# filodb/FiloDB

Measured on NVIDIA H100. Metric: samples/s scanned+aggregated (rate over 10M series); % HBM roofline, higher is better.
Workload: dtype f64

## Files before the change

filodb_b200/csrc/capi.cu:

```cuda
#include "../../include/filo_b200.h"
#include "kernels.h"
#include "host_util.h"
#include "scan_tile_layout.h"
#include "scan_wp_layout.h"
#include <cub/cub.cuh>
#include <algorithm>
#include <atomic>
#include <chrono>
#include <cmath>
#include <cstdio>
#include <cstdlib>
#include <cstring>
#include <mutex>
#include <string>
#include <thread>
#include <vector>

using namespace filo;

struct filo_ctx {
  int device = 0;
  filo_cfg cfg{};
  cudaStream_t stream = nullptr;
  int sm_count = 132;
// ... 776 lines not shown
  CUDA_TRY(ctx, tmp.alloc((void**)&d_err, 16)); CUDA_TRY(ctx, tmp.alloc((void**)&d_counters, 16));
  CUDA_TRY(ctx, cudaMemsetAsync(d_err, 0, 16, s)); CUDA_TRY(ctx, cudaMemsetAsync(d_counters, 0, 16, s));
  EventPair evp;
  if (stats) { CUDA_TRY(ctx, cudaEventCreate(&evp.e0)); CUDA_TRY(ctx, cudaEventCreate(&evp.e1)); }
  cudaEvent_t& e0 = evp.e0; cudaEvent_t& e1 = evp.e1;

  const uint32_t acc_bytes = fused ? align_up((uint32_t)q.T * (moments ? 20u : 12u), 128) : 0;
  const bool need_corr2 = need_corr && t->any_drop;
  uint32_t scratch2 = align_up((uint32_t)t->max_chunks * (uint32_t)CHUNK_DESC_BYTES, 16) +
                      ((uint32_t)t->max_rows + (uint32_t)t->max_chunks * 8u) * 8u * (1u + (t->any_nonconst_ts ? 1u : 0u) + (need_corr2 ? 1u : 0u));
  scratch2 = align_up(scratch2 + 16, 128);
  const uint32_t rec_cap = align_up(t->max_rec_bytes + 16, 128);
  const size_t per_warp2 = v2_smem_per_warp(rec_cap, scratch2, acc_bytes);
  const char* force_env = std::getenv("FILO_KERNEL");
  const std::string force = force_env ? force_env : "";
  const size_t smem_cap = std::min<size_t>(ctx->max_smem_optin, 227 * 1024);
  const bool use_v2 = force != "v1" && t->max_rec_bytes > 0 && per_warp2 * FAST_WARPS + 1024 <= smem_cap;
  const int64_t work = fused ? t->n_items : t->n_series;
  int64_t launches = 0;
  uint8_t* gscratch = nullptr;
  ScanLaunch L{t->d_arena, t->d_rec_off, t->n_series, q, nullptr, 0, 0, d_counters, d_err, 1, s};
  uint32_t rec_cap_used = 0;
  if (use_v2) {
    const size_t cta_smem = per_warp2 * FAST_WARPS + 1024;
    const int ctas_per_sm = (int)std::max<size_t>(1, std::min<size_t>(64 / FAST_WARPS, (size_t)(228 * 1024) / cta_smem));
    L.grid = (int)std::max<int64_t>(1, std::min<int64_t>((work + FAST_WARPS - 1) / FAST_WARPS, (int64_t)ctx->sm_count * ctas_per_sm));
    L.scratch_bytes = scratch2; L.use_smem = 1; rec_cap_used = rec_cap;
  } else {
    uint32_t scratch = align_up((uint32_t)t->max_chunks * (uint32_t)CHUNK_DESC_BYTES, 16) + (uint32_t)t->max_rows * 8u * (need_corr ? 3u : 2u);
    scratch = align_up(scratch + 16, 16);
    const size_t cta_smem = (size_t)(scratch + acc_bytes) * SCAN_WARPS;
    const int use_smem = cta_smem <= std::min<size_t>(ctx->max_smem_optin, 200 * 1024);
    int ctas_per_sm = 16;
    if (use_smem) ctas_per_sm = (int)std::max<size_t>(1, std::min<size_t>(16, (size_t)(220 * 1024) / std::max<size_t>(cta_smem + 1024, 1)));
    L.grid = (int)std::max<int64_t>(1, std::min<int64_t>((work + SCAN_WARPS - 1) / SCAN_WARPS, (int64_t)ctx->sm_count * ctas_per_sm));
    if (!use_smem) CUDA_TRY(ctx, tmp.alloc((void**)&gscratch, (size_t)L.grid * SCAN_WARPS * (scratch + acc_bytes)));
    L.gscratch = gscratch; L.scratch_bytes = scratch; L.use_smem = use_smem;
  }
  const int fn_cls = fn_class_of(fn, q.cumulative, q.long_values);
  const uint64_t wrows = (uint64_t)(q.window / q.step) + 1;
  TileSmem TL{};
  bool use_tile = false;
  if (use_v2 && force != "v2" && fn_cls == CLASS_SUM && t->n_series > 0) {
    TL = tile_layout(t->max_rec_bytes, (uint32_t)t->max_rows, (uint32_t)q.T, (uint32_t)std::min<uint64_t>(2 * wrows, 1u << 20) + 16);
    if (((size_t)TL.total + 1024) * 2 > (size_t)228 * 1024) TL = tile_layout(t->max_rec_bytes, (uint32_t)t->max_rows, (uint32_t)q.T, 16);
    use_tile = (size_t)TL.total + 1024 <= smem_cap;
  }
  WpSmem WL{};
  bool use_wp = false;
  if (use_tile && force != "v3" && wrows <= 4096 && t->max_chunks > 0) {
    const bool alias = wp_max_items((uint32_t)t->max_chunks, (uint32_t)q.T, (uint32_t)wrows) <= 64;
    WL = wp_layout(t->max_rec_bytes, (uint32_t)t->max_rows, (uint32_t)t->max_chunks, (uint32_t)q.T, (uint32_t)wrows, alias);
    WL.warps = (uint32_t)std::min<size_t>(smem_cap / WL.per_warp, alias ? WP_MAX_WARPS_ALIAS : WP_MAX_WARPS);
    use_wp = WL.warps >= 4;
  }
  WpCtrSmem WC{};
  bool use_wp_ctr = false;
  if (use_v2 && force != "v2" && force != "v3" && fn_cls == CLASS_COUNTER && t->n_series > 0 && t->max_chunks > 0 &&
      (!fused || q.T <= TILE_AGG_ACC * TILE_THREADS) && wp_ctr_tile_footprint_ok(t->max_rec_bytes, (uint32_t)t->max_rows, (uint32_t)q.T, smem_cap)) {
    WC = wp_ctr_layout(t->max_rec_bytes, (uint32_t)t->max_rows, (uint32_t)t->max_chunks, (uint32_t)q.T, fused, t->any_nonconst_ts, moments);
    const size_t w = std::min<size_t>((smem_cap - sizeof(TileCtrTab) * (TILE_CTR_TABMAX + 1) - 64) / WC.per_warp, WC.tsr != 0 ? 16 : WP_CTR_MAX_WARPS);
    WC.warps = (uint32_t)w; WC.tab = (uint32_t)(WC.per_warp * w);
    use_wp_ctr = w >= 4;
  }
  auto run_per_series = [&](double* outp) -> int32_t {
    if (use_tile || use_wp_ctr) {
      int64_t* d_list = nullptr; unsigned long long* d_cnt = nullptr;
      CUDA_TRY(ctx, tmp.alloc((void**)&d_list, (size_t)t->n_series * 8));
      CUDA_TRY(ctx, tmp.alloc((void**)&d_cnt, 16));
      CUDA_TRY(ctx, cudaMemsetAsync(d_cnt, 0, 16, s));
      ScanLaunch LT = L;
      static const bool dbg = std::getenv("FILO_DEBUG_SYNC") != nullptr;
      if (use_wp) {
        LT.grid = (int)std::max<int64_t>(1, std::min<int64_t>((t->n_series + WL.warps - 1) / WL.warps, (int64_t)ctx->sm_count));
        CUDA_TRY(ctx, launch_scan_wp(LT, outp, WL, d_list, d_cnt));
      } else if (use_wp_ctr) {
        LT.grid = (int)std::max<int64_t>(1, std::min<int64_t>((t->n_series + WC.warps - 1) / WC.warps, (int64_t)ctx->sm_count));
        CUDA_TRY(ctx, launch_scan_wp_ctr(LT, outp, WC, d_list, d_cnt));
      } else {
        const int ctas_per_sm = ((size_t)TL.total + 1024) * 2 <= (size_t)228 * 1024 ? 2 : 1;
        const int64_t n_tiles = (t->n_series + TILE_NS - 1) / TILE_NS;
        LT.grid = (int)std::max<int64_t>(1, std::min<int64_t>(n_tiles, (int64_t)ctx->sm_count * ctas_per_sm));
        if (dbg) { fprintf(stderr, "[filo] tile kernel fn=%d T=%d grid=%d smem=%u pitch=%u\n", fn, q.T, LT.grid, TL.total, TL.vals_pitch); fflush(stderr); }
        CUDA_TRY(ctx, launch_scan_tile(LT, outp, TL, d_list, d_cnt));
      }
      if (dbg) { CUDA_TRY(ctx, cudaStreamSynchronize(s)); fprintf(stderr, "[filo] tile kernel done\n"); fflush(stderr); }
      ScanLaunch LF = L; LF.list = d_list; LF.list_count = d_cnt;
      CUDA_TRY(ctx, launch_scan_series_v2(LF, outp, rec_cap_used));
      if (dbg) { CUDA_TRY(ctx, cudaStreamSynchronize(s)); fprintf(stderr, "[filo] fallback kernel done\n"); fflush(stderr); }
      launches += 2;
    } else {
      CUDA_TRY(ctx, use_v2 ? launch_scan_series_v2(L, outp, rec_cap_used) : launch_scan_series(L, outp));
      launches += 1;
    }
    return FILO_OK;
  };
  if (stats) CUDA_TRY(ctx, cudaEventRecord(e0, s));
  if (agg == FILO_AGG_NONE) {
    { int32_t rc = run_per_series((double*)d_out_values); if (rc) return rc; }
  } else if (!fused) {
    double* per = nullptr;
    CUDA_TRY(ctx, tmp.alloc((void**)&per, (size_t)t->n_series * q.T * 8));
    { int32_t rc = run_per_series(per); if (rc) return rc; }
    CUDA_TRY(ctx, launch_topk(per, t->grouped ? t->d_order : nullptr, t->d_group_start, t->n_groups, q.T, k, agg == FILO_AGG_BOTTOMK,
                              (double*)d_out_values, (int64_t*)d_out_aux, s));
    launches += 1;
// ... 541 lines not shown
```

filodb_b200/csrc/scan_wp.cuh:

```cuda
#pragma once
#include "scan_tile.cuh"
#include "scan_wp_layout.h"

namespace filo {

#ifdef FILO_CUSIM
__device__ __forceinline__ uint32_t wp_soff(const void* p) { return (uint32_t)(reinterpret_cast<const uint8_t*>(p) - smem); }
__device__ __forceinline__ uint32_t wp_lds32(uint32_t off) { uint32_t v; std::memcpy(&v, smem + off, 4); return v; }
#else
__device__ __forceinline__ uint32_t wp_soff(const void* p) { return smem_u32(p); }
__device__ __forceinline__ uint32_t wp_lds32(uint32_t off) { uint32_t v; asm volatile("ld.shared.u32 %0, [%1];" : "=r"(v) : "r"(off)); return v; }
#endif

#if defined(FILO_WP_PROF) && !defined(FILO_CUSIM)
__device__ unsigned long long g_wp_prof[16];
#define WPROF_DECL uint32_t wpp_t0 = (uint32_t)clock(), wpp_acc[14] = {0, 0, 0, 0, 0, 0, 0, 0, 0, 0, 0, 0, 0, 0};
#define WPROF(i) { const uint32_t wpp_t1 = (uint32_t)clock(); wpp_acc[i] += wpp_t1 - wpp_t0; wpp_t0 = wpp_t1; }
#define WPROF_COUNT(i) { ++wpp_acc[i]; }
#define WPROF_FLUSH if (lane == 0) { for (int wpp_i = 0; wpp_i < 14; ++wpp_i) atomicAdd(&g_wp_prof[wpp_i], (unsigned long long)wpp_acc[wpp_i]); atomicAdd(&g_wp_prof[15], 1ull); }
#else
#define WPROF_DECL
#define WPROF(i)
#define WPROF_COUNT(i)
#define WPROF_FLUSH
// ... 237 lines not shown

constexpr uint32_t WP_FINAL = 0, WP_RAWFIN = 1, WP_JUNC = 2, WP_GAP = 3;
__device__ __forceinline__ int wp_chunk_of(const WpChunk* CD, int n, int k) {
  int ci = -1;
  for (int c = 0; c < n; ++c) if (CD[c].nblk > 0 && k >= CD[c].kT0) ci = c;
  return ci;
}
__device__ __forceinline__ uint32_t wp_class(const WpChunk* CD, int n, int k, uint32_t& jslot) {
  const int ci = wp_chunk_of(CD, n, k);
  jslot = 0;
  if (ci < 0 || k > CD[ci].kT1) return WP_GAP;
  const WpChunk& ch = CD[ci];
  const int i = k - ch.kT0;
  if (i < ch.jzb * WP_R) { jslot = (uint32_t)(ch.joff + i) | (i < ch.hs ? 128u : 0u); return WP_JUNC; }
  return i >= ch.tb * WP_R ? WP_RAWFIN : WP_FINAL;
}
__device__ __forceinline__ int wp_rows_in(const WpChunk& x, int k, int Wr) {
  int lo = x.s0 + k; if (lo < 0) lo = 0; int hi = x.s0 + k + Wr; if (hi > x.nrows - 1) hi = x.nrows - 1;
  return hi - lo + 1;
}

__device__ __forceinline__ void wp_item(const WpChunk* CD, const WpSmem& L, int it, int items, int psi, int& pp, int& op, int& inf) {
  const bool active = it < items;
  int ci = 0;
  if (CD[1].nblk > 0 && it >= CD[1].blk0) ci = 1;
  if (CD[2].nblk > 0 && it >= CD[2].blk0) ci = 2;
  if (CD[3].nblk > 0 && it >= CD[3].blk0) ci = 3;
  const WpChunk& ch = CD[ci];
  const int b = active ? it - ch.blk0 : 0;
  const int k0 = ch.kT0 + WP_R * b;
  pp = ch.vidx0 + 9 * b;
  const bool tojz = b < ch.jzb;
  const bool raw = tojz || b >= ch.tb;
  op = tojz ? (int)WP_OFF_J + 8 * (ch.joff + WP_R * b) : (int)L.out + 8 * (k0 + ((k0 + psi) >> 3));
  int jEnd = !active ? -1 : tojz ? WP_R - 1 : ch.kT1 - k0;
  if (jEnd > WP_R - 1) jEnd = WP_R - 1;
  const int ot = tojz ? 0 : (k0 + psi) & 7;
  inf = (jEnd + 1) | ((raw ? 1 : 0) << 4) | (ot << 5) | (ci << 8) | (k0 << 10);
}

template <int FN, int NW>
__global__ void __launch_bounds__(NW * 32, 1)
scan_wp_sum_kernel(const uint8_t* __restrict__ arena, const int64_t* __restrict__ rec_off, int64_t n_series, QueryParams q,
                   double* __restrict__ out, WpSmem L, int64_t* __restrict__ fallback_list, unsigned long long* __restrict__ fallback_count,
                   unsigned long long* d_counters, int* d_err) {
  extern __shared__ __align__(128) uint8_t smem[];
  const unsigned FULL = 0xffffffffu;
  const int lane = threadIdx.x & 31, warp = threadIdx.x >> 5;
  uint8_t* wb = smem + (size_t)warp * L.per_warp;
  uint64_t* bar = reinterpret_cast<uint64_t*>(wb);
  WpChunk* CD = reinterpret_cast<WpChunk*>(wb + WP_OFF_DESC);
  uint64_t* xtab = reinterpret_cast<uint64_t*>(wb + WP_OFF_J);
  double* J = reinterpret_cast<double*>(wb + WP_OFF_J);
  uint8_t* R = wb + WP_OFF_REC;
  double* V = reinterpret_cast<double*>(wb + L.vals);
  double* O = reinterpret_cast<double*>(wb + L.out);
  const int64_t nwarps = (int64_t)gridDim.x * (blockDim.x >> 5);
  int64_t s = (int64_t)blockIdx.x * (blockDim.x >> 5) + warp;
  if (lane == 0) { mbar_init(bar, 1); mbar_fence_init(); }
  __syncwarp();

  int64_t winDur = q.inclusive ? q.window : q.window - 1; if (winDur < 0) winDur = 0;
  const double fdiv = (double)(q.inclusive ? winDur : winDur + 1), frcp = 1.0 / fdiv;
  const int64_t S0 = q.start - winDur, E0 = q.start;
  const int64_t lastEnd = q.start + (int64_t)(q.T - 1) * q.step;
  StepDiv sd; sd.init(q.step);
  const double NaNv = __longlong_as_double(0x7ff8000000000000LL);

  int64_t m_init = 0, m_end = 0; int m_nrows = -1, m_n = -1, m_wire = -1; bool m_ok = false;
  int dd_dst[2] = {0, 0}, dd_inf[2] = {0, 0}, wi_pp[2] = {0, 0}, wi_op[2] = {0, 0}, wi_inf[2] = {0, 0};
  int gz[3] = {-1, -1, -1}; bool gz_all = true;
  int p_Wr = 0, p_items = 0, p_nfull = 0, p_psi = 0; double p_rcpn = 0.0; bool p_oal = false;
  uint32_t p_cls = 0; uint64_t p_jx = 0;
  int64_t rows_scanned = 0, bytes_scanned = 0;
  uint32_t parity = 0;

  auto issue = [&](int64_t off, uint32_t sz) {
    mbar_expect_tx(bar, sz);
    tma_load_1d(R, arena + off, sz, bar);
  };
  int64_t cur_off = 0; uint32_t cur_sz = 0;
  if (s < n_series) { cur_off = rec_off[s]; cur_sz = (uint32_t)(rec_off[s + 1] - cur_off); }
  if (s < n_series && cur_sz <= L.rec_cap && lane == 0) issue(cur_off, cur_sz);
  WPROF_DECL

  for (; s < n_series; s += nwarps) {
    const int64_t sn = s + nwarps;
    int64_t nxt_off = 0; uint32_t nxt_end = 0;
    if (sn < n_series) { nxt_off = rec_off[sn]; nxt_end = (uint32_t)rec_off[sn + 1]; }
    const bool staged = cur_sz <= L.rec_cap;
    WPROF_COUNT(10)
    WPROF(9)
    if (staged) { mbar_wait(bar, parity); parity ^= 1; }
    WPROF(0)
    const WpParsed P = wp_parse<true>(R, q, staged, lane);
    const uint32_t nxt_sz = nxt_end - (uint32_t)nxt_off;
    WPROF(1)
    bool regular = P.regular;
    const bool have = P.have; const int n = P.n, c = lane;
    const int64_t init = P.init, end_time = P.end_time;
    const int nrows = P.nrows, num_rows = P.num_rows, vbytes = P.vbytes, ng = P.ng, vwire = P.vwire, grp_base = P.grp_base, ngroups = P.ngroups;
    const uint32_t voff = P.voff, w12 = P.w12; const bool any_raw = P.any_raw;
    const bool samec = !(c < n) || (init == m_init && nrows == m_nrows && end_time == m_end && vwire == m_wire);
    const bool same_all = __all_sync(FULL, samec);
    const bool same = m_ok && n == m_n && same_all;
    if (regular && !same) {
      WPROF_COUNT(11)
      m_init = init; m_end = end_time; m_nrows = nrows; m_n = n; m_wire = vwire; m_ok = false;
      int64_t s0 = 0, e0 = 0;
      if (have) { s0 = sd.ceil_div(S0 - init); e0 = sd.floor_div(E0 - init); }
      const int Wr = (int)(e0 - s0);
      int64_t kT0 = -e0; if (kT0 < 0) kT0 = 0;
      int64_t kT1 = (int64_t)(nrows - 1) - s0; if (kT1 > q.T - 1) kT1 = q.T - 1;
      const bool touch = have && kT0 <= kT1;
      if (!touch) { kT0 = 0x3fffffff; kT1 = -1; }
      const int Wr0 = __shfl_sync(FULL, Wr, 0);
      bool okp = !have || Wr == Wr0;
      if (Wr0 < 8 || (uint32_t)Wr0 + 1 > L.jcap) okp = false;
      const unsigned tm = __ballot_sync(FULL, touch) & 0xfu;
      if (tm != 0) { const unsigned lowbit = tm & (0u - tm); const unsigned filled = tm + lowbit; if ((filled & (filled - 1)) != 0) okp = false; }
      const int64_t kT1p = __shfl_up_sync(FULL, kT1, 1), kT1pp = __shfl_up_sync(FULL, kT1, 2), kT0n = __shfl_down_sync(FULL, kT0, 1);
      const bool prev_t = c > 0 && ((tm >> (c - 1)) & 1u), next_t = c + 1 < WP_MAXC && ((tm >> (c + 1)) & 1u);
      if (touch && c >= 2 && ((tm >> (c - 2)) & 1u) && !(kT1pp < kT0)) okp = false;
      int64_t ownLo = kT0, ownHi = kT1;
      if (touch && prev_t && kT1p + 1 > ownLo) ownLo = kT1p + 1;
      if (touch && next_t && kT0n - 1 < ownHi) ownHi = kT0n - 1;
      const int hs = touch ? (int)(ownLo - kT0) : 0;
      const int nblk = touch ? (int)((kT1 - kT0 + WP_R) / WP_R) : 0;
      const int jzb = (hs + WP_R - 1) / WP_R;
      const int tb = (touch && ownHi < kT1) ? (int)((ownHi + 1 - kT0) / WP_R) : nblk;
      if (touch && jzb > tb) okp = false;
      int blk0, items, joff, jtot;
      { const int a0 = __shfl_sync(FULL, nblk, 0), a1 = __shfl_sync(FULL, nblk, 1), a2 = __shfl_sync(FULL, nblk, 2), a3 = __shfl_sync(FULL, nblk, 3);
        blk0 = (c > 0 ? a0 : 0) + (c > 1 ? a1 : 0) + (c > 2 ? a2 : 0); items = a0 + a1 + a2 + a3; }
      { const int z = jzb * WP_R;
        const int a0 = __shfl_sync(FULL, z, 0), a1 = __shfl_sync(FULL, z, 1), a2 = __shfl_sync(FULL, z, 2), a3 = __shfl_sync(FULL, z, 3);
        joff = (c > 0 ? a0 : 0) + (c > 1 ? a1 : 0) + (c > 2 ? a2 : 0); jtot = a0 + a1 + a2 + a3; }
      if ((uint32_t)jtot > L.jcap) okp = false;
      if (L.alias && items > 64) okp = false;
      const int fr = touch ? (int)(s0 + kT0) : 0;
      int rowpos = 0;
      {
        int base = 0;
#pragma unroll
        for (int cc = 0; cc < WP_MAXC; ++cc) {
          int x;
// ... 17 lines not shown
          p_psi = (-(int)__shfl_sync(FULL, (int)(touch ? kT0 : 0), first_t)) & 7;
          p_oal = __all_sync(FULL, !touch || (((int)kT0 + p_psi) & 7) == 0); }
        p_Wr = Wr0; p_items = items; p_nfull = Wr0 + 1; p_rcpn = 1.0 / (double)(Wr0 + 1);
        __syncwarp();
        {
          int tot = 0;
          gz[0] = gz[1] = gz[2] = -1;
          for (int g = 0; g <= n; ++g) {
            const int g0 = g == 0 ? 0 : CD[g - 1].rowpos + CD[g - 1].nrows;
            const int g1 = g == n ? pend : CD[g].rowpos;
#pragma unroll
            for (int u = 0; u < 3; ++u) { const int i = u * 32 + lane - tot; if (i >= 0 && i < g1 - g0) gz[u] = wp_vidx(g0 + i); }
            tot += g1 - g0;
          }
          gz_all = tot <= 96;
        }
        {
          uint32_t cls = 0; uint64_t jx = 0; int nj = 0;
#pragma unroll 1
          for (int m = 0; m < 16 && lane + 32 * m < q.T; ++m) {
            uint32_t js;
            const uint32_t code = wp_class(CD, n, lane + 32 * m, js);
            cls |= code << (2 * m);
            if (code == WP_JUNC) { jx |= (uint64_t)js << (8 * nj); ++nj; }
          }
          p_cls = cls; p_jx = jx;
        }
        {
          const int gb1 = __shfl_sync(FULL, have ? grp_base : 0x7fffffff, 1), gb2 = __shfl_sync(FULL, have ? grp_base : 0x7fffffff, 2),
                    gb3 = __shfl_sync(FULL, have ? grp_base : 0x7fffffff, 3);
#pragma unroll
          for (int jj = 0; jj < 2; ++jj) {
            const int slot = jj * 32 + lane;
            const bool active = slot < ngroups;
            const int ci = active ? (slot >= gb1 ? 1 : 0) + (slot >= gb2 ? 1 : 0) + (slot >= gb3 ? 1 : 0) : 0;
            const int gbc = ci == 0 ? 0 : ci == 1 ? gb1 : ci == 2 ? gb2 : gb3;
            const int g = active ? slot - gbc : 0;
            const int pq = CD[ci].rowpos + 1 + g * 8;
            dd_dst[jj] = wp_vidx(pq);
            dd_inf[jj] = (active ? 1 : 0) | (ci << 1) | ((pq & 7) << 3) | (g << 8);
          }
#pragma unroll
          for (int X = 0; X < 2; ++X) wp_item(CD, L, X * 32 + lane, items, p_psi, wi_pp[X], wi_op[X], wi_inf[X]);
        }
        m_ok = true;
      }
    }
    WPROF(2)
    if (!regular) {
      WPROF_COUNT(12)
      if (lane == 0) { const unsigned long long slot = atomicAdd(fallback_count, 1ull); fallback_list[slot] = s; }
      __syncwarp();
      if (sn < n_series && nxt_sz <= L.rec_cap && lane == 0) issue(nxt_off, nxt_sz);
      cur_off = nxt_off; cur_sz = nxt_sz;
      continue;
    }
    if (c < WP_MAXC) {
      WpChunk& d = CD[c];
      d.grp_base = have ? grp_base : 0x7fffffff; d.ng = ng; d.wire = vwire; d.val_off = voff; d.dropped = P.dropped;
      if (have && vwire == WIRE_XOR) { const uint32_t po = w12 >> 16; d.first = ld64(R + voff + po); d.grp_off = voff + po + 8; d.tab_off = voff + XOR_OFF_GROUPTAB; }
      else { d.first = have ? ld64(R + voff + 8) : 0ull; d.grp_off = 0; d.tab_off = 0; }
    }
    int cnt_rows = 0, cnt_bytes = 0;
    { const int64_t endp = __shfl_up_sync(FULL, end_time, 1);
      if (have && !(c > 0 && !(endp < lastEnd))) { cnt_rows = num_rows; cnt_bytes = vbytes; } }
#pragma unroll
    for (int o = 1; o < WP_MAXC; o <<= 1) { cnt_rows += __shfl_xor_sync(FULL, cnt_rows, o); cnt_bytes += __shfl_xor_sync(FULL, cnt_bytes, o); }
    __syncwarp();
    WPROF(3)
    auto rec_done = [&]() {
      __syncwarp();
      if (sn < n_series && nxt_sz <= L.rec_cap && lane == 0) issue(nxt_off, nxt_sz);
    };
    const uint32_t okbits = wp_decode<false>(R, V, CD, xtab, dd_dst, dd_inf, n, any_raw, lane, nullptr, rec_done);
    const bool vals_ok = __all_sync(FULL, (okbits >> 30) & 1u);
    __syncwarp();
    cur_off = nxt_off; cur_sz = nxt_sz;
    WPROF(4)
    if (gz_all) {
#pragma unroll
      for (int u = 0; u < 3; ++u) if (gz[u] >= 0) V[gz[u]] = 0.0;
    } else {
      const int pend = CD[n - 1].rowpos + CD[n - 1].nrows + p_Wr + 8;
      for (int g = 0; g <= n; ++g) {
        const int g0 = g == 0 ? 0 : CD[g - 1].rowpos + CD[g - 1].nrows;
        const int g1 = g == n ? pend : CD[g].rowpos;
        for (int pz = g0 + lane; pz < g1; pz += 32) V[wp_vidx(pz)] = 0.0;
      }
    }
    WPROF(5)
    if (!vals_ok) {
      WPROF_COUNT(13)
      if (lane == 0) { const unsigned long long slot = atomicAdd(fallback_count, 1ull); fallback_list[slot] = s; }
      __syncwarp();
      continue;
    }
    if (lane == 0) { rows_scanned += cnt_rows; bytes_scanned += cnt_bytes; }
    __syncwarp();
    const int psi = p_psi;
    auto oidx = [&](int k) -> int { return k + ((k + psi) >> 3); };
    {
      const int Wr = p_Wr;
      for (int it0 = 0; it0 < p_items; it0 += 64) {
        int ipp[2], iop[2], iinf[2];
#pragma unroll
        for (int X = 0; X < 2; ++X) {
          if (it0 == 0) { ipp[X] = wi_pp[X]; iop[X] = wi_op[X]; iinf[X] = wi_inf[X]; }
          else wp_item(CD, L, it0 + X * 32 + lane, p_items, psi, ipp[X], iop[X], iinf[X]);
        }
        const double* pp[2]; double* op[2]; int jEnd[2], ot[2]; bool rawm[2];
#pragma unroll
        for (int X = 0; X < 2; ++X) {
          pp[X] = V + ipp[X]; op[X] = reinterpret_cast<double*>(wb + iop[X]);
          jEnd[X] = (iinf[X] & 15) - 1; rawm[X] = (iinf[X] >> 4) & 1; ot[X] = (iinf[X] >> 5) & 7;
        }
        double a[WP_R], bb[WP_R];
        wp_block_pair(pp[0], pp[1], Wr, a, bb);
        __syncwarp();
#pragma unroll
        for (int X = 0; X < 2; ++X) {
          const double dv = rawm[X] ? 1.0 : fdiv, rc = rawm[X] ? 1.0 : frcp, sc = rawm[X] ? 1.0 : 1000.0;
#pragma unroll
          for (int j = 0; j < WP_R; ++j) {
            const double raw = X ? bb[j] : a[j];
            int nn = 1;
            if (FN == FN_AVG || FN == FN_COUNT) {
              const WpChunk& ch = CD[(iinf[X] >> 8) & 3];
              int lo = ch.s0 + (iinf[X] >> 10) + j; const int hi0 = lo + Wr; if (lo < 0) lo = 0;
              const int hi = hi0 > ch.nrows - 1 ? ch.nrows - 1 : hi0;
              nn = hi - lo + 1;
// ... 70 lines not shown
```

filodb_b200/csrc/scan_wp_layout.h:

```cpp
#pragma once
#include <stdint.h>
#include "filo_record.h"
#include "scan_params.h"
#include "scan_tile_layout.h"
namespace filo {
constexpr int WP_MAXC = 4;
constexpr int WP_MAXG = 64;
constexpr int WP_R = 8;
constexpr int WP_MAX_WARPS = 16;
constexpr int WP_MAX_WARPS_ALIAS = 20;

struct WpChunk {
  uint64_t first;
  int32_t kT0, kT1;
  int32_t ownLo, ownHi;
  int32_t blk0, nblk;
  int32_t vidx0;
  int32_t rowpos;
  int32_t nrows, s0, e0;
  int32_t grp_base, ng, wire;
  uint32_t grp_off, tab_off, val_off;
  int32_t joff, hs;
  int32_t jzb, tb;
  int32_t dropped;
};
static_assert(sizeof(WpChunk) == 96, "WpChunk");

constexpr uint32_t WP_OFF_DESC = 16, WP_OFF_J = WP_OFF_DESC + WP_MAXC * 96, WP_J_DOUBLES = 128, WP_OFF_REC = WP_OFF_J + WP_J_DOUBLES * 8;
struct WpSmem {
  uint32_t desc, jbuf, rec, vals, out, per_warp;
  uint32_t rec_cap, vcap , jcap , ocap ;
  uint32_t warps;
  uint32_t alias;
};
FILO_HD inline WpSmem wp_layout(uint32_t max_rec_bytes, uint32_t max_rows, uint32_t max_chunks, uint32_t T, uint32_t wrows, bool alias) {
  WpSmem L;
  if (max_chunks > (uint32_t)WP_MAXC) max_chunks = WP_MAXC;
  L.rec_cap = align_up(max_rec_bytes + 16, 16);
  const uint32_t P = max_rows + (max_chunks + 1) * (wrows + 7) + 16;
  L.vcap = align_up(P + P / 8 + 2, 2);
  L.jcap = WP_J_DOUBLES;
  (void)wrows;
  L.ocap = align_up(T + T / 8 + 4, 2);
  if (alias && L.vcap < L.ocap) L.vcap = L.ocap;
  static_assert(sizeof(WpChunk) == 96, "WP_OFF_J");
  uint32_t o = WP_OFF_REC;
  L.desc = WP_OFF_DESC; L.jbuf = WP_OFF_J;
  L.rec = o; o += L.rec_cap;
  L.vals = o; o += L.vcap * 8;
  if (alias) L.out = L.vals; else { L.out = o; o += L.ocap * 8; }
  L.per_warp = align_up(o, 16);
  L.warps = 0;
  L.alias = alias ? 1u : 0u;
  return L;
}
FILO_HD inline uint32_t wp_max_items(uint32_t max_chunks, uint32_t T, uint32_t wrows) {
  if (max_chunks > (uint32_t)WP_MAXC) max_chunks = WP_MAXC;
  if (max_chunks == 0) max_chunks = 1;
  return (T + (max_chunks - 1) * (wrows - 1) + 7 * max_chunks) / 8;
}

constexpr int WP_CTR_MAX_WARPS = 20;
struct TileCtr {
  double dTS, thr, half, endpart, sI, ratio0, skipC;
  int32_t dropped, pad;
};
constexpr int TILE_MAXDROP = 8;
constexpr int TILE_CTR_TABMAX = 64;
struct TileCtrTab { double sI, thr, half, rcpSI; };
struct TileDrops {
  int32_t n, pos[TILE_MAXDROP], pad[3];
  double amt[TILE_MAXDROP];
};
struct WpCtrChunk {
  int64_t init, end_time;
  int32_t nrows, s0, e0, rowpos;
  int32_t kA, kB;
  int32_t kA2, kB2;
  TileCtr kc;
};
static_assert(sizeof(WpCtrChunk) == 112, "WpCtrChunk");

struct WpCtrSmem {
  uint32_t vals, kc, acc, nbad, per_warp, tab ;
  uint32_t rec_cap, vcap , warps, agg;
  uint32_t tsr;
};
constexpr uint32_t WP_OFF_DROPS = WP_OFF_J + 64 * 8;
static_assert(WP_OFF_DROPS + WP_MAXC * sizeof(TileDrops) <= WP_OFF_REC, "drops fit in front of the record");
FILO_HD inline WpCtrSmem wp_ctr_layout(uint32_t max_rec_bytes, uint32_t max_rows, uint32_t max_chunks, uint32_t T, bool agg, bool irr = false,
                                       bool moments = false) {
  WpCtrSmem L;
  if (max_chunks > (uint32_t)WP_MAXC) max_chunks = WP_MAXC;
  L.rec_cap = align_up(max_rec_bytes + 16, 16);
  const uint32_t P = max_rows + 8 * max_chunks + 8;
  L.vcap = align_up(P + P / 8 + 2, 2);
  uint32_t o = WP_OFF_REC + L.rec_cap;
  L.vals = o; o += L.vcap * 8;
  L.kc = o; o += (uint32_t)(WP_MAXC * sizeof(WpCtrChunk));
  L.tsr = 0;
  if (irr) { L.tsr = o; o += align_up(P * 4, 16); }
// ... 15 lines not shown
```

scratch/c2_ceiling.py:

```python
import ctypes as C
import json
import os
import statistics
import subprocess
import sys
import tempfile

READ_B, WRITE_B = 3762, 3848
SRC = r"""
#include <cstdint>
#include <cuda_runtime.h>
__global__ void __launch_bounds__(640) c2_copy(const uint4* __restrict__ src, double* __restrict__ dst, long long rows) {
  const int lane = threadIdx.x & 31;
  const long long nw = (long long)gridDim.x * (blockDim.x >> 5);
  for (long long s = (long long)blockIdx.x * (blockDim.x >> 5) + (threadIdx.x >> 5); s < rows; s += nw) {
    // row s reads the 16-byte words that start inside its bytes [s * 3762, (s + 1) * 3762): the words of all rows tile the buffer
    const long long w0 = (s * 3762 + 15) / 16, w1 = ((s + 1) * 3762 + 15) / 16;
    unsigned long long acc = 0;
    for (long long w = w0 + lane; w < w1; w += 32) { const uint4 v = __ldcs(src + w); acc ^= ((unsigned long long)v.x | ((unsigned long long)v.y << 32)) ^ v.z ^ ((unsigned long long)v.w << 17); }
    double* o = dst + s * 481;
    for (int i = lane; i < 481; i += 32) __stcs(o + i, (double)(acc + (unsigned long long)i));
  }
}
extern "C" int c2_run(long long rows, int warmup, int reps, float* ms_out, char* name, int name_len) {
  cudaDeviceProp p; if (cudaGetDeviceProperties(&p, 0) != cudaSuccess) return -1;
  for (int i = 0; i < name_len - 1 && p.name[i]; ++i) { name[i] = p.name[i]; name[i + 1] = 0; }
  const size_t rb = (size_t)rows * 3762 + 64, wb = (size_t)rows * 3848;
  uint4* src = nullptr; double* dst = nullptr;
  if (cudaMalloc(&src, rb) != cudaSuccess) return -2;
  if (cudaMalloc(&dst, wb) != cudaSuccess) { cudaFree(src); return -3; }
  cudaMemset(src, 0x5a, rb);
  const int grid = p.multiProcessorCount;                     // one persistent CTA of 20 warps per SM, as the C2 kernel runs
  cudaEvent_t a, b; cudaEventCreate(&a); cudaEventCreate(&b);
  for (int i = 0; i < warmup; ++i) c2_copy<<<grid, 640>>>(src, dst, rows);
  for (int i = 0; i < reps; ++i) {
    cudaEventRecord(a); c2_copy<<<grid, 640>>>(src, dst, rows); cudaEventRecord(b); cudaEventSynchronize(b);
    cudaEventElapsedTime(ms_out + i, a, b);
  }
  const cudaError_t e = cudaGetLastError();
  cudaEventDestroy(a); cudaEventDestroy(b); cudaFree(src); cudaFree(dst);
  return e == cudaSuccess ? 0 : -4;
}
"""


def smi():
    q = "name,power.limit,clocks.max.sm,clocks.sm"
    try:
        r = subprocess.run(["nvidia-smi", "--query-gpu=" + q, "--format=csv,noheader", "-i", "0"], capture_output=True, text=True, timeout=30)
        return dict(zip(q.split(","), [x.strip() for x in r.stdout.strip().split(",")]))
    except (OSError, subprocess.SubprocessError):
        return {}


def main():
    rows = int(sys.argv[1]) if len(sys.argv) > 1 else 5_000_000
    tmp = tempfile.mkdtemp(prefix="c2_ceiling_")
    cu, so = os.path.join(tmp, "c2_copy.cu"), os.path.join(tmp, "c2_copy.so")
    with open(cu, "w") as f:
        f.write(SRC)
    subprocess.run(["nvcc", "-gencode", "arch=compute_90a,code=sm_90a", "-O3", "-shared", "-Xcompiler", "-fPIC", cu, "-o", so], check=True)
    lib = C.CDLL(so)
    reps = 10
    ms = (C.c_float * reps)()
    name = C.create_string_buffer(128)
    before = smi()
    rc = lib.c2_run(C.c_longlong(rows), 3, reps, ms, name, 128)
    after = smi()
    if rc != 0:
        raise SystemExit("c2_ceiling: CUDA error %d (no GPU, or not enough memory for %d rows)" % (rc, rows))
    t = sorted(ms)
    rd, wr = rows * READ_B, rows * WRITE_B
    med = statistics.median(t)
    res = {"gpu": name.value.decode(), "smi_before": before, "smi_after": after, "rows": rows, "read_bytes": rd, "write_bytes": wr,
           "ms_min": t[0], "ms_median": med, "ms_max": t[-1], "tb_per_s_median": (rd + wr) / (med * 1e-3) / 1e12}
    res["share_of_3_35_tb_s"] = res["tb_per_s_median"] / 3.35
    print("%s, power limit %s, max SM clock %s (SM clock %s after the runs)" % (res["gpu"], after.get("power.limit", "?"),
          after.get("clocks.max.sm", "?"), after.get("clocks.sm", "?")))
    print("C2 byte mix (%d rows: read %.1f GB, write %.1f GB): %.2f ms median (%.2f-%.2f over %d runs), %.2f TB/s = %.0f %% of 3.35 TB/s"
          % (rows, rd / 1e9, wr / 1e9, med, t[0], t[-1], reps, res["tb_per_s_median"], 100 * res["share_of_3_35_tb_s"]))
    if len(sys.argv) > 2:
        with open(sys.argv[2], "w") as f:
            json.dump(res, f, indent=1)


if __name__ == "__main__":
    main()
```

Before: 143.7 billion.

## Double-buffer per-warp TMA record staging in the windowed sum scan kernel

Adds a second per-warp record buffer and mbarrier to the wp sum kernel, so each warp keeps two series' records in flight via cp.async.bulk. The host picks this layout only when shared memory still fits the maximum warp count. The aim is to hide HBM load latency behind decode and aggregation of the current series, at the cost of more shared memory per warp. The scratch bandwidth-ceiling script is also expanded into a survey of several copy shapes, which is a measurement tool only.

```diff
diff --git a/filodb_b200/csrc/capi.cu b/filodb_b200/csrc/capi.cu
--- a/filodb_b200/csrc/capi.cu
+++ b/filodb_b200/csrc/capi.cu
@@ -852,6 +852,8 @@
     const bool alias = wp_max_items((uint32_t)t->max_chunks, (uint32_t)q.T, (uint32_t)wrows) <= 64;
     WL = wp_layout(t->max_rec_bytes, (uint32_t)t->max_rows, (uint32_t)t->max_chunks, (uint32_t)q.T, (uint32_t)wrows, alias);
     WL.warps = (uint32_t)std::min<size_t>(smem_cap / WL.per_warp, alias ? WP_MAX_WARPS_ALIAS : WP_MAX_WARPS);
+    const WpSmem WL2 = wp_layout(t->max_rec_bytes, (uint32_t)t->max_rows, (uint32_t)t->max_chunks, (uint32_t)q.T, (uint32_t)wrows, alias, true);
+    if (smem_cap / WL2.per_warp >= (size_t)WP_MAX_WARPS) { WL = WL2; WL.warps = WP_MAX_WARPS; }
     use_wp = WL.warps >= 4;
   }
   WpCtrSmem WC{};
diff --git a/filodb_b200/csrc/scan_wp.cuh b/filodb_b200/csrc/scan_wp.cuh
--- a/filodb_b200/csrc/scan_wp.cuh
+++ b/filodb_b200/csrc/scan_wp.cuh
@@ -313,12 +313,13 @@
   WpChunk* CD = reinterpret_cast<WpChunk*>(wb + WP_OFF_DESC);
   uint64_t* xtab = reinterpret_cast<uint64_t*>(wb + WP_OFF_J);
   double* J = reinterpret_cast<double*>(wb + WP_OFF_J);
+  const bool two = L.rec2 != 0;
   uint8_t* R = wb + WP_OFF_REC;
   double* V = reinterpret_cast<double*>(wb + L.vals);
   double* O = reinterpret_cast<double*>(wb + L.out);
   const int64_t nwarps = (int64_t)gridDim.x * (blockDim.x >> 5);
   int64_t s = (int64_t)blockIdx.x * (blockDim.x >> 5) + warp;
-  if (lane == 0) { mbar_init(bar, 1); mbar_fence_init(); }
+  if (lane == 0) { mbar_init(bar, 1); if (two) mbar_init(bar + 1, 1); mbar_fence_init(); }
   __syncwarp();
 
   int64_t winDur = q.inclusive ? q.window : q.window - 1; if (winDur < 0) winDur = 0;
@@ -337,22 +338,31 @@
   uint32_t parity = 0;
 
   auto issue = [&](int64_t off, uint32_t sz) {
-    mbar_expect_tx(bar, sz);
-    tma_load_1d(R, arena + off, sz, bar);
+    uint64_t* b = bar + (R == wb + WP_OFF_REC ? 0 : 1);
+    mbar_expect_tx(b, sz);
+    tma_load_1d(R, arena + off, sz, b);
   };
-  int64_t cur_off = 0; uint32_t cur_sz = 0;
+  uint32_t cur_sz = 0, nb_sz = 0;
+  int64_t cur_off = 0;
   if (s < n_series) { cur_off = rec_off[s]; cur_sz = (uint32_t)(rec_off[s + 1] - cur_off); }
   if (s < n_series && cur_sz <= L.rec_cap && lane == 0) issue(cur_off, cur_sz);
+  if (two && s + nwarps < n_series) {
+    const int64_t o1 = rec_off[s + nwarps]; nb_sz = (uint32_t)(rec_off[s + nwarps + 1] - o1);
+    R = wb + L.rec2;
+    if (nb_sz <= L.rec_cap && lane == 0) issue(o1, nb_sz);
+    R = wb + WP_OFF_REC;
+  }
+  uint32_t stage = 0;
   WPROF_DECL
 
   for (; s < n_series; s += nwarps) {
-    const int64_t sn = s + nwarps;
+    const int64_t sn = s + (two ? 2 : 1) * nwarps;
     int64_t nxt_off = 0; uint32_t nxt_end = 0;
     if (sn < n_series) { nxt_off = rec_off[sn]; nxt_end = (uint32_t)rec_off[sn + 1]; }
     const bool staged = cur_sz <= L.rec_cap;
     WPROF_COUNT(10)
     WPROF(9)
-    if (staged) { mbar_wait(bar, parity); parity ^= 1; }
+    if (staged) { mbar_wait(bar + stage, (parity >> stage) & 1u); parity ^= 1u << stage; }
     WPROF(0)
     const WpParsed P = wp_parse<true>(R, q, staged, lane);
     const uint32_t nxt_sz = nxt_end - (uint32_t)nxt_off;
@@ -476,7 +486,7 @@
       if (lane == 0) { const unsigned long long slot = atomicAdd(fallback_count, 1ull); fallback_list[slot] = s; }
       __syncwarp();
       if (sn < n_series && nxt_sz <= L.rec_cap && lane == 0) issue(nxt_off, nxt_sz);
-      cur_off = nxt_off; cur_sz = nxt_sz;
+      if (two) { cur_sz = nb_sz; nb_sz = nxt_sz; stage ^= 1u; R = wb + (stage ? L.rec2 : WP_OFF_REC); } else cur_sz = nxt_sz;
       continue;
     }
     if (c < WP_MAXC) {
@@ -499,7 +509,7 @@
     const uint32_t okbits = wp_decode<false>(R, V, CD, xtab, dd_dst, dd_inf, n, any_raw, lane, nullptr, rec_done);
     const bool vals_ok = __all_sync(FULL, (okbits >> 30) & 1u);
     __syncwarp();
-    cur_off = nxt_off; cur_sz = nxt_sz;
+    if (two) { cur_sz = nb_sz; nb_sz = nxt_sz; stage ^= 1u; R = wb + (stage ? L.rec2 : WP_OFF_REC); } else cur_sz = nxt_sz;
     WPROF(4)
     if (gz_all) {
 #pragma unroll
diff --git a/filodb_b200/csrc/scan_wp_layout.h b/filodb_b200/csrc/scan_wp_layout.h
--- a/filodb_b200/csrc/scan_wp_layout.h
+++ b/filodb_b200/csrc/scan_wp_layout.h
@@ -32,8 +32,9 @@
   uint32_t rec_cap, vcap , jcap , ocap ;
   uint32_t warps;
   uint32_t alias;
+  uint32_t rec2;
 };
-FILO_HD inline WpSmem wp_layout(uint32_t max_rec_bytes, uint32_t max_rows, uint32_t max_chunks, uint32_t T, uint32_t wrows, bool alias) {
+FILO_HD inline WpSmem wp_layout(uint32_t max_rec_bytes, uint32_t max_rows, uint32_t max_chunks, uint32_t T, uint32_t wrows, bool alias, bool two_rec = false) {
   WpSmem L;
   if (max_chunks > (uint32_t)WP_MAXC) max_chunks = WP_MAXC;
   L.rec_cap = align_up(max_rec_bytes + 16, 16);
@@ -47,6 +48,8 @@
   uint32_t o = WP_OFF_REC;
   L.desc = WP_OFF_DESC; L.jbuf = WP_OFF_J;
   L.rec = o; o += L.rec_cap;
+  L.rec2 = 0;
+  if (two_rec) { L.rec2 = o; o += L.rec_cap; }
   L.vals = o; o += L.vcap * 8;
   if (alias) L.out = L.vals; else { L.out = o; o += L.ocap * 8; }
   L.per_warp = align_up(o, 16);
diff --git a/scratch/c2_ceiling.py b/scratch/c2_ceiling.py
--- a/scratch/c2_ceiling.py
+++ b/scratch/c2_ceiling.py
@@ -7,36 +7,237 @@
 import tempfile
 
 READ_B, WRITE_B = 3762, 3848
+SHAPES = ["copy", "read", "write", "pf_l2", "pair_v2", "warp_tma2", "bulk8_s3", "bulk4_s3x2", "copy_v2", "warp_tma1", "warp_tma1_v2",
+          "warp_tma2_v2"]
 SRC = r"""
 #include <cstdint>
 #include <cuda_runtime.h>
-__global__ void __launch_bounds__(640) c2_copy(const uint4* __restrict__ src, double* __restrict__ dst, long long rows) {
+#define RB 3762LL
+#define NT 481
+
+__device__ __forceinline__ unsigned long long mix(uint4 v) { return ((unsigned long long)v.x | ((unsigned long long)v.y << 32)) ^ v.z ^ ((unsigned long long)v.w << 17); }
+// row s reads the 16-byte words that start inside its bytes [s * 3762, (s + 1) * 3762): the words of all rows tile the buffer
+__device__ __forceinline__ long long w_lo(long long s) { return (s * RB + 15) / 16; }
+__device__ __forceinline__ uint32_t sa(const void* p) { return (uint32_t)__cvta_generic_to_shared(p); }
+__device__ __forceinline__ void bar_init(uint64_t* b) {
+  asm volatile("mbarrier.init.shared::cta.b64 [%0], 1;" ::"r"(sa(b)) : "memory");
+  asm volatile("fence.mbarrier_init.release.cluster;" ::: "memory");
+  asm volatile("fence.proxy.async.shared::cta;" ::: "memory");
+}
+__device__ __forceinline__ void bulk_load(void* d, const void* g, uint32_t bytes, uint64_t* b) {
+  asm volatile("mbarrier.arrive.expect_tx.shared::cta.b64 _, [%0], %1;" ::"r"(sa(b)), "r"(bytes) : "memory");
+  asm volatile("cp.async.bulk.shared::cluster.global.mbarrier::complete_tx::bytes [%0], [%1], %2, [%3];"
+               ::"r"(sa(d)), "l"(g), "r"(bytes), "r"(sa(b)) : "memory");
+}
+__device__ __forceinline__ void bar_wait(uint64_t* b, uint32_t parity) {
+  uint32_t ok;
+  do {
+    asm volatile("{\n\t.reg .pred p;\n\tmbarrier.try_wait.parity.shared::cta.b64 p, [%1], %2;\n\tselp.u32 %0, 1, 0, p;\n\t}"
+                 : "=r"(ok) : "r"(sa(b)), "r"(parity) : "memory");
+  } while (!ok);
+}
+
+__global__ void __launch_bounds__(640) c2_copy(const uint4* __restrict__ src, double* __restrict__ dst, long long rows, int pf) {
   const int lane = threadIdx.x & 31;
   const long long nw = (long long)gridDim.x * (blockDim.x >> 5);
   for (long long s = (long long)blockIdx.x * (blockDim.x >> 5) + (threadIdx.x >> 5); s < rows; s += nw) {
-    // row s reads the 16-byte words that start inside its bytes [s * 3762, (s + 1) * 3762): the words of all rows tile the buffer
-    const long long w0 = (s * 3762 + 15) / 16, w1 = ((s + 1) * 3762 + 15) / 16;
-    unsigned long long acc = 0;
-    for (long long w = w0 + lane; w < w1; w += 32) { const uint4 v = __ldcs(src + w); acc ^= ((unsigned long long)v.x | ((unsigned long long)v.y << 32)) ^ v.z ^ ((unsigned long long)v.w << 17); }
-    double* o = dst + s * 481;
-    for (int i = lane; i < 481; i += 32) __stcs(o + i, (double)(acc + (unsigned long long)i));
-  }
-}
-extern "C" int c2_run(long long rows, int warmup, int reps, float* ms_out, char* name, int name_len) {
+    if (pf && lane == 0 && s + 2 * nw < rows) {
+      const long long a = w_lo(s + 2 * nw), b = w_lo(s + 2 * nw + 1);
+      asm volatile("cp.async.bulk.prefetch.L2.global [%0], %1;" ::"l"(src + a), "r"((uint32_t)(b - a) * 16u) : "memory");
+    }
+    const long long w0 = w_lo(s), w1 = w_lo(s + 1);
+    unsigned long long acc = 0;
+    for (long long w = w0 + lane; w < w1; w += 32) acc ^= mix(__ldcs(src + w));
+    double* o = dst + s * NT;
+    for (int i = lane; i < NT; i += 32) __stcs(o + i, (double)(acc + (unsigned long long)i + 1));
+  }
+}
+
+__global__ void __launch_bounds__(640) c2_read(const uint4* __restrict__ src, double* __restrict__ dst, long long rows) {
+  const int lane = threadIdx.x & 31;
+  const long long nw = (long long)gridDim.x * (blockDim.x >> 5);
+  unsigned long long acc = 0;
+  for (long long s = (long long)blockIdx.x * (blockDim.x >> 5) + (threadIdx.x >> 5); s < rows; s += nw)
+    for (long long w = w_lo(s) + lane, w1 = w_lo(s + 1); w < w1; w += 32) acc ^= mix(__ldcs(src + w));
+  if (acc == 0x0123456789abcdefull) dst[threadIdx.x] = (double)acc;         // never true for the data the survey writes
+}
+
+__global__ void __launch_bounds__(640) c2_write(const uint4* __restrict__ src, double* __restrict__ dst, long long rows) {
+  const int lane = threadIdx.x & 31;
+  const long long nw = (long long)gridDim.x * (blockDim.x >> 5);
+  for (long long s = (long long)blockIdx.x * (blockDim.x >> 5) + (threadIdx.x >> 5); s < rows; s += nw) {
+    double* o = dst + s * NT;
+    for (int i = lane; i < NT; i += 32) __stcs(o + i, (double)(s + i + 1));
+  }
+}
+
+__global__ void __launch_bounds__(640) c2_pair(const uint4* __restrict__ src, double* __restrict__ dst, long long rows) {
+  const int lane = threadIdx.x & 31;
+  const long long nw = (long long)gridDim.x * (blockDim.x >> 5), np = rows / 2;
+  for (long long p = (long long)blockIdx.x * (blockDim.x >> 5) + (threadIdx.x >> 5); p < np; p += nw) {
+    const long long w0 = w_lo(2 * p), w1 = w_lo(2 * p + 2);
+    unsigned long long acc = 0;
+    for (long long w = w0 + lane; w < w1; w += 32) acc ^= mix(__ldcs(src + w));
+    double2* o = reinterpret_cast<double2*>(dst + 2 * p * NT);                 // 2 * 481 * 8 = 7,696 = 16 * 481: 16-byte aligned
+    for (int i = lane; i < NT; i += 32) __stcs(o + i, make_double2((double)(acc + 2 * i + 1), (double)(acc + 2 * i + 2)));
+  }
+}
+
+// 481 results of row s from 16-byte-aligned stores: row s starts at 8 mod 16 when s is odd, so its window 0 is stored alone and
+// windows (2j - 1, 2j) in pairs; an even row stores windows (2j, 2j + 1) in pairs and its window 480 alone
+__device__ __forceinline__ void row_v2(double* dst, long long s, unsigned long long acc, int lane) {
+  const int h = (int)(s & 1);
+  double2* vb = reinterpret_cast<double2*>(dst + s * NT - h);                 // virtual window v = k + h; v = 2j, 2j + 1 at vb[j]
+  for (int j = lane; j <= NT / 2; j += 32) {
+    const double lo = (double)(acc + 2 * j + 1), hi = (double)(acc + 2 * j + 2);
+    const bool vlo = 2 * j >= h, vhi = 2 * j + 1 < NT + h;
+    if (vlo && vhi) __stcs(vb + j, make_double2(lo, hi));
+    else if (vlo) __stcs(reinterpret_cast<double*>(vb + j), lo);
+    else if (vhi) __stcs(reinterpret_cast<double*>(vb + j) + 1, hi);
+  }
+}
+
+__global__ void __launch_bounds__(640) c2_copy_v2(const uint4* __restrict__ src, double* __restrict__ dst, long long rows) {
+  const int lane = threadIdx.x & 31;
+  const long long nw = (long long)gridDim.x * (blockDim.x >> 5);
+  for (long long s = (long long)blockIdx.x * (blockDim.x >> 5) + (threadIdx.x >> 5); s < rows; s += nw) {
+    unsigned long long acc = 0;
+    for (long long w = w_lo(s) + lane, w1 = w_lo(s + 1); w < w1; w += 32) acc ^= mix(__ldcs(src + w));
+    row_v2(dst, s, acc, lane);
+  }
+}
+
+// one warp per row, each row fetched into the warp's shared memory by one cp.async.bulk, NB rows in flight per warp (NB x 3,808 B
+// + the mbarriers); the next copy is issued as soon as the row is read, before its results are stored (as the C2 kernel does)
+#define WT_BUF 3808
+template <int NB, bool V2>
+__global__ void __launch_bounds__(640) c2_warp_tma(const uint4* __restrict__ src, double* __restrict__ dst, long long rows) {
+  extern __shared__ __align__(128) uint8_t sm[];
+  const int lane = threadIdx.x & 31, warp = threadIdx.x >> 5;
+  uint8_t* base = sm + (size_t)warp * (NB * WT_BUF + 16);
+  uint64_t* bar = reinterpret_cast<uint64_t*>(base + NB * WT_BUF);
+  const long long nw = (long long)gridDim.x * (blockDim.x >> 5);
+  long long s = (long long)blockIdx.x * (blockDim.x >> 5) + warp;
+  if (lane == 0) for (int j = 0; j < NB; ++j) bar_init(bar + j);
+  __syncwarp();
+  for (int j = 0; j < NB; ++j)
+    if (lane == 0 && s + j * nw < rows) { const long long a = w_lo(s + j * nw); bulk_load(base + j * WT_BUF, src + a, (uint32_t)(w_lo(s + j * nw + 1) - a) * 16u, bar + j); }
+  for (int it = 0; s < rows; s += nw, ++it) {
+    const int st = it % NB;
+    bar_wait(bar + st, (uint32_t)(it / NB) & 1u);
+    const long long w0 = w_lo(s), w1 = w_lo(s + 1);
+    const uint4* r = reinterpret_cast<const uint4*>(base + st * WT_BUF);
+    unsigned long long acc = 0;
+    for (int w = lane; w < (int)(w1 - w0); w += 32) acc ^= mix(r[w]);
+    __syncwarp();
+    if (lane == 0 && s + NB * nw < rows) { const long long a = w_lo(s + NB * nw); bulk_load(base + st * WT_BUF, src + a, (uint32_t)(w_lo(s + NB * nw + 1) - a) * 16u, bar + st); }
+    if (V2) row_v2(dst, s, acc, lane);
+    else { double* o = dst + s * NT; for (int i = lane; i < NT; i += 32) __stcs(o + i, (double)(acc + (unsigned long long)i + 1)); }
+  }
+}
+
+// CTA-cooperative: batches of B consecutive rows, ST loads and OST stores in flight; warp w of the CTA takes row w of a batch
+template <int B, int ST, int OST>
+__global__ void __launch_bounds__(B * 32) c2_bulk(const uint4* __restrict__ src, double* __restrict__ dst, long long rows) {
+  constexpr int LB = ((B * 3762 + 32 + 15) / 16) * 16, OB = B * NT * 8;
+  extern __shared__ __align__(128) uint8_t sm[];
+  uint8_t* ld = sm;                                   // ST x LB
+  double* ob = reinterpret_cast<double*>(sm + ST * LB); // OST x OB
+  uint64_t* bar = reinterpret_cast<uint64_t*>(sm + ST * LB + OST * OB);
+  const int lane = threadIdx.x & 31, warp = threadIdx.x >> 5;
+  const long long nb = rows / B;
+  auto issue = [&](long long b, int st) {
+    const long long a = b * B * RB / 16, e = ((b + 1) * B * RB + 15) / 16;
+    bulk_load(ld + st * LB, src + a, (uint32_t)(e - a) * 16u, bar + st);
+  };
+  if (threadIdx.x == 0) { for (int i = 0; i < ST; ++i) bar_init(bar + i); }
+  __syncthreads();
+  if (threadIdx.x == 0)
+    for (int j = 0; j < ST; ++j) if (blockIdx.x + (long long)j * gridDim.x < nb) issue(blockIdx.x + (long long)j * gridDim.x, j);
+  int j = 0;
+  for (long long b = blockIdx.x; b < nb; b += gridDim.x, ++j) {
+    const int st = j % ST, os = j % OST;
+    bar_wait(bar + st, (uint32_t)(j / ST) & 1u);
+    if (threadIdx.x == 0) asm volatile("cp.async.bulk.wait_group.read %0;" ::"n"(OST - 1) : "memory");   // store j - OST has left ob[os]
+    __syncthreads();
+    const long long s = b * B + warp, a = b * B * RB / 16;
+    const uint4* r = reinterpret_cast<const uint4*>(ld + st * LB);
+    unsigned long long acc = 0;
+    for (long long w = w_lo(s) + lane, w1 = w_lo(s + 1); w < w1; w += 32) acc ^= mix(r[w - a]);
+    double* o = ob + (size_t)os * (B * NT) + warp * NT;
+    for (int i = lane; i < NT; i += 32) o[i] = (double)(acc + (unsigned long long)i + 1);
+    asm volatile("fence.proxy.async.shared::cta;" ::: "memory");
+    __syncthreads();
+    if (threadIdx.x == 0) {
+      asm volatile("cp.async.bulk.global.shared::cta.bulk_group [%0], [%1], %2;" ::"l"(dst + b * B * NT), "r"(sa(ob + (size_t)os * (B * NT))), "r"((uint32_t)OB) : "memory");
+      asm volatile("cp.async.bulk.commit_group;" ::: "memory");
+      if (b + (long long)ST * gridDim.x < nb) issue(b + (long long)ST * gridDim.x, st);
+    }
+  }
+  if (threadIdx.x == 0) asm volatile("cp.async.bulk.wait_group 0;" ::: "memory");
+}
+template <int B, int ST, int OST> constexpr int bulk_smem() { return ST * (((B * 3762 + 32 + 15) / 16) * 16) + OST * B * NT * 8 + 8 * ST; }
+
+// shape k, one launch
+static int launch(int k, int sms, const uint4* src, double* dst, long long rows) {
+  switch (k) {
+    case 0: c2_copy<<<sms, 640>>>(src, dst, rows, 0); break;
+    case 1: c2_read<<<sms, 640>>>(src, dst, rows); break;
+    case 2: c2_write<<<sms, 640>>>(src, dst, rows); break;
+    case 3: c2_copy<<<sms, 640>>>(src, dst, rows, 1); break;
+    case 4: c2_pair<<<sms, 640>>>(src, dst, rows); break;
+    case 5: c2_warp_tma<2, false><<<sms, 640, 20 * (2 * WT_BUF + 16)>>>(src, dst, rows); break;
+    case 6: c2_bulk<8, 3, 2><<<sms, 256, bulk_smem<8, 3, 2>()>>>(src, dst, rows); break;
+    case 7: c2_bulk<4, 3, 2><<<2 * sms, 128, bulk_smem<4, 3, 2>()>>>(src, dst, rows); break;
+    case 8: c2_copy_v2<<<sms, 640>>>(src, dst, rows); break;
+    case 9: c2_warp_tma<1, false><<<sms, 640, 20 * (WT_BUF + 16)>>>(src, dst, rows); break;
+    case 10: c2_warp_tma<1, true><<<sms, 640, 20 * (WT_BUF + 16)>>>(src, dst, rows); break;
+    case 11: c2_warp_tma<2, true><<<sms, 640, 20 * (2 * WT_BUF + 16)>>>(src, dst, rows); break;
+    default: return -1;
+  }
+  return 0;
+}
+
+// nshapes shapes, `reps` rounds of one launch each (after `warmup` rounds): ms_out[k * reps + i].  Before the rounds, every shape
+// that stores results runs once on a zeroed output and `check_out[k]` counts the sampled result slots it left at zero.
+extern "C" int c2_run(long long rows, int nshapes, int warmup, int reps, float* ms_out, long long* check_out, char* name, int name_len) {
   cudaDeviceProp p; if (cudaGetDeviceProperties(&p, 0) != cudaSuccess) return -1;
   for (int i = 0; i < name_len - 1 && p.name[i]; ++i) { name[i] = p.name[i]; name[i + 1] = 0; }
+  if (rows % 8 != 0) return -5;                       // the bulk shapes store whole batches
   const size_t rb = (size_t)rows * 3762 + 64, wb = (size_t)rows * 3848;
   uint4* src = nullptr; double* dst = nullptr;
   if (cudaMalloc(&src, rb) != cudaSuccess) return -2;
   if (cudaMalloc(&dst, wb) != cudaSuccess) { cudaFree(src); return -3; }
   cudaMemset(src, 0x5a, rb);
-  const int grid = p.multiProcessorCount;                     // one persistent CTA of 20 warps per SM, as the C2 kernel runs
+  cudaFuncSetAttribute(c2_warp_tma<2, false>, cudaFuncAttributeMaxDynamicSharedMemorySize, 20 * (2 * WT_BUF + 16));
+  cudaFuncSetAttribute(c2_warp_tma<2, true>, cudaFuncAttributeMaxDynamicSharedMemorySize, 20 * (2 * WT_BUF + 16));
+  cudaFuncSetAttribute(c2_warp_tma<1, false>, cudaFuncAttributeMaxDynamicSharedMemorySize, 20 * (WT_BUF + 16));
+  cudaFuncSetAttribute(c2_warp_tma<1, true>, cudaFuncAttributeMaxDynamicSharedMemorySize, 20 * (WT_BUF + 16));
+  cudaFuncSetAttribute(c2_bulk<8, 3, 2>, cudaFuncAttributeMaxDynamicSharedMemorySize, bulk_smem<8, 3, 2>());
+  cudaFuncSetAttribute(c2_bulk<4, 3, 2>, cudaFuncAttributeMaxDynamicSharedMemorySize, bulk_smem<4, 3, 2>());
+  const int sms = p.multiProcessorCount;
+  for (int k = 0; k < nshapes; ++k) {
+    check_out[k] = -1;
+    if (k == 1) continue;
+    cudaMemset(dst, 0, wb);
+    if (launch(k, sms, src, dst, rows) != 0) return -6;
+    if (cudaGetLastError() != cudaSuccess || cudaDeviceSynchronize() != cudaSuccess) return -100 - k;
+    long long zeros = 0;
+    for (int i = 0; i < 4096; ++i) {                  // spread over the rows, both parities, first and last slots included
+      const long long r = i == 4095 ? rows - 1 : (long long)((unsigned long long)i * 2654435761ull % (unsigned long long)rows);
+      const int c = i % 3 == 0 ? 0 : i % 3 == 1 ? NT - 1 : (i * 37) % NT;
+      double v = 0.0; cudaMemcpy(&v, dst + r * NT + c, 8, cudaMemcpyDeviceToHost);
+      zeros += v == 0.0;
+    }
+    check_out[k] = zeros;
+  }
   cudaEvent_t a, b; cudaEventCreate(&a); cudaEventCreate(&b);
-  for (int i = 0; i < warmup; ++i) c2_copy<<<grid, 640>>>(src, dst, rows);
-  for (int i = 0; i < reps; ++i) {
-    cudaEventRecord(a); c2_copy<<<grid, 640>>>(src, dst, rows); cudaEventRecord(b); cudaEventSynchronize(b);
-    cudaEventElapsedTime(ms_out + i, a, b);
-  }
+  for (int i = 0; i < warmup; ++i) for (int k = 0; k < nshapes; ++k) launch(k, sms, src, dst, rows);
+  for (int i = 0; i < reps; ++i)
+    for (int k = 0; k < nshapes; ++k) {
+      cudaEventRecord(a); launch(k, sms, src, dst, rows); cudaEventRecord(b); cudaEventSynchronize(b);
+      cudaEventElapsedTime(ms_out + k * reps + i, a, b);
+    }
   const cudaError_t e = cudaGetLastError();
   cudaEventDestroy(a); cudaEventDestroy(b); cudaFree(src); cudaFree(dst);
   return e == cudaSuccess ? 0 : -4;
@@ -61,24 +262,31 @@
         f.write(SRC)
     subprocess.run(["nvcc", "-gencode", "arch=compute_90a,code=sm_90a", "-O3", "-shared", "-Xcompiler", "-fPIC", cu, "-o", so], check=True)
     lib = C.CDLL(so)
-    reps = 10
-    ms = (C.c_float * reps)()
+    reps, ns = 10, len(SHAPES)
+    ms = (C.c_float * (reps * ns))()
+    chk = (C.c_longlong * ns)()
     name = C.create_string_buffer(128)
     before = smi()
-    rc = lib.c2_run(C.c_longlong(rows), 3, reps, ms, name, 128)
+    rc = lib.c2_run(C.c_longlong(rows), ns, 2, reps, ms, chk, name, 128)
     after = smi()
     if rc != 0:
-        raise SystemExit("c2_ceiling: CUDA error %d (no GPU, or not enough memory for %d rows)" % (rc, rows))
-    t = sorted(ms)
+        raise SystemExit("c2_ceiling: CUDA error %d (no GPU, rows not a multiple of 8, not enough memory for %d rows, or -100 - k: shape k "
+                         "did not run)" % (rc, rows))
     rd, wr = rows * READ_B, rows * WRITE_B
-    med = statistics.median(t)
     res = {"gpu": name.value.decode(), "smi_before": before, "smi_after": after, "rows": rows, "read_bytes": rd, "write_bytes": wr,
-           "ms_min": t[0], "ms_median": med, "ms_max": t[-1], "tb_per_s_median": (rd + wr) / (med * 1e-3) / 1e12}
-    res["share_of_3_35_tb_s"] = res["tb_per_s_median"] / 3.35
-    print("%s, power limit %s, max SM clock %s (SM clock %s after the runs)" % (res["gpu"], after.get("power.limit", "?"),
-          after.get("clocks.max.sm", "?"), after.get("clocks.sm", "?")))
-    print("C2 byte mix (%d rows: read %.1f GB, write %.1f GB): %.2f ms median (%.2f-%.2f over %d runs), %.2f TB/s = %.0f %% of 3.35 TB/s"
-          % (rows, rd / 1e9, wr / 1e9, med, t[0], t[-1], reps, res["tb_per_s_median"], 100 * res["share_of_3_35_tb_s"]))
+           "reps": reps, "shapes": {}}
+    print("%s, power limit %s, max SM clock %s (SM clock %s before, %s after the runs)" % (res["gpu"], after.get("power.limit", "?"),
+          after.get("clocks.max.sm", "?"), before.get("clocks.sm", "?"), after.get("clocks.sm", "?")))
+    print("%d rows: read %.1f GB, write %.1f GB; %d alternated rounds" % (rows, rd / 1e9, wr / 1e9, reps))
+    for k, sh in enumerate(SHAPES):
+        t = sorted(ms[k * reps:(k + 1) * reps])
+        med = statistics.median(t)
+        by = (rd if sh != "write" else 0) + (wr if sh != "read" else 0)
+        tbs = by / (med * 1e-3) / 1e12
+        res["shapes"][sh] = {"ms": list(ms[k * reps:(k + 1) * reps]), "ms_min": t[0], "ms_median": med, "ms_max": t[-1], "bytes": by,
+                             "tb_per_s_median": tbs, "share_of_3_35_tb_s": tbs / 3.35, "sampled_zero_results": chk[k]}
+        print("  %-11s %7.2f ms median (%.2f-%.2f)  %5.2f TB/s = %3.0f %% of 3.35 TB/s%s" % (sh, med, t[0], t[-1], tbs, 100 * tbs / 3.35,
+              "" if chk[k] <= 0 else "  CHECK FAILED: %d of 4096 sampled results not written" % chk[k]))
     if len(sys.argv) > 2:
         with open(sys.argv[2], "w") as f:
             json.dump(res, f, indent=1)
```

After: 152.0 billion, median of 6. +5.8%, better.
